# av-savchenko/HSE_FaceRec_tf

Hardware: AMD Instinct MI355X
Metric: faces/sec embedding-extract (MobileNet-192, bs=256) (higher is better)
Workload: dtype f32

## Files before the change

hse_facerec_tf_amd/csrc/dwpw_f16s.hip:

```cpp
#include <type_traits>

#include "common.h"

namespace hsefr {

namespace {

typedef float f32x4 __attribute__((ext_vector_type(4)));
typedef float f32x16 __attribute__((ext_vector_type(16)));
typedef _Float16 f16x4 __attribute__((ext_vector_type(4)));
typedef _Float16 f16x8 __attribute__((ext_vector_type(8)));

struct DwPwSParams {
    const float4* x;
    const float4* wd;
    const float4* dscale;
    const float4* dshift;
    const float* wsplit;
    const float* descale;
    const float* pshift;
    float* y;
    int H, W, C4, KT, OH, OW, Cout, pad_t, pad_l, tiles_w, tiles_h, tiles_n;
    unsigned total;
    float a_scale;
    int reverse;
    int nimg;
    unsigned m_n, m_w, m_h;
    int rows, seam;
    unsigned m_seam;
    unsigned long long* stamps;
};

constexpr int ROWB = 128;
__device__ __forceinline__ int swzb(int row, int chunk) { return row * ROWB + 16 * (chunk ^ ((row >> 1) & 7) ^ ((row & 1) << 2)); }
__device__ __forceinline__ float4 fma4(float4 a, float4 b, float4 c) {
    return make_float4(fmaf(a.x, b.x, c.x), fmaf(a.y, b.y, c.y), fmaf(a.z, b.z, c.z), fmaf(a.w, b.w, c.w));
}
__device__ __forceinline__ float relu6(float v) { return fminf(fmaxf(v, 0.f), 6.f); }
__device__ __forceinline__ unsigned fastdiv(unsigned x, unsigned m) { return m ? __umulhi(x, m) : x; }

template <int STRIDE, int TW, int BN, int OCC, int ACT>
__global__ __launch_bounds__(256, OCC) void dwpw_f16s_kernel(DwPwSParams p) {
    constexpr int TH = 128 / TW;
    constexpr int U = TW * 8;
    constexpr int RG = 256 / U;
    constexpr int RPT = TH / RG;
    static_assert(RPT == 4, "patch shapes 8x16 and 16x8");
    constexpr int WN = BN / 2, NI = WN / 32, BP = BN / 32;
    __shared__ __attribute__((aligned(16))) unsigned char As[128 * ROWB];
    __shared__ __attribute__((aligned(16))) unsigned char Bs[BN * ROWB];

    const int tid = threadIdx.x;
    const int lane = tid & 63, wave = tid >> 6;
    const int wm = wave >> 1, wn = wave & 1;
    const int li = lane & 31, lh = lane >> 5;
    const int srow = tid >> 3, skq = tid & 7;
    const int u = tid % U, tw = u >> 3, c4l = u & 7;
    const int row0 = (tid / U) * RPT;
    const int arow = wm * 64 + li, brow = wn * WN + li;

    for (unsigned t = blockIdx.x; t < p.total; t += gridDim.x) {
        const unsigned lt = xcd_remap_dir(t, p.total, p.reverse);
        const int n0 = (lt % p.tiles_n) * BN;
        const unsigned pt = lt / p.tiles_n;
        const int ow0 = (pt % p.tiles_w) * TW;
        const int oh0 = ((pt / p.tiles_w) % p.tiles_h) * TH;
        const int n = pt / (p.tiles_w * p.tiles_h);

        const int ow = min(ow0 + tw, p.OW - 1);
        const int iw0 = ow * STRIDE - p.pad_l;
        const float ml = iw0 >= 0 ? 1.f : 0.f, mm = (iw0 + 1 >= 0 && iw0 + 1 < p.W) ? 1.f : 0.f, mr = iw0 + 2 < p.W ? 1.f : 0.f;
        const int cl = max(iw0, 0) * p.C4, cm = min(max(iw0 + 1, 0), p.W - 1) * p.C4, cr = min(iw0 + 2, p.W - 1) * p.C4;
        const float4* ximg = p.x + (size_t)n * p.H * p.W * p.C4;
        const int ih0 = (oh0 + row0) * STRIDE - p.pad_t;
        const float* bsrc = p.wsplit + (size_t)(n0 + srow) * p.KT * 32 + 4 * skq;

        f32x16 acc[2][NI];
#pragma unroll
        for (int mi = 0; mi < 2; ++mi)
#pragma unroll
            for (int ni = 0; ni < NI; ++ni)
#pragma unroll
                for (int r = 0; r < 16; ++r) acc[mi][ni][r] = 0.f;

        for (int kc = 0; kc < p.KT; ++kc) {
            f32x4 rb[BP];
#pragma unroll
            for (int q = 0; q < BP; ++q) rb[q] = *(const f32x4*)(bsrc + (size_t)32 * q * p.KT * 32 + kc * 32);
            const int c4 = kc * 8 + c4l;
            const float4* xin = ximg + c4;
            float4 wk[9];
#pragma unroll
            for (int i = 0; i < 9; ++i) {
                const float m = (i % 3 == 0) ? ml : (i % 3 == 1 ? mm : mr);
                const float4 wr = p.wd[i * p.C4 + c4];
                wk[i] = make_float4(wr.x * m, wr.y * m, wr.z * m, wr.w * m);
            }
            const float4 dsc = p.dscale[c4], dsh = p.dshift[c4];
            struct Row { float4 l, m, r; float k; };
            auto load_row = [&](int ih) {
                Row q;
                const int ihc = min(max(ih, 0), p.H - 1);
                const float4* row = xin + (size_t)ihc * p.W * p.C4;
                q.l = row[cl]; q.m = row[cm]; q.r = row[cr];
                q.k = (ih >= 0 && ih < p.H) ? 1.f : 0.f;
                return q;
            };
            auto row_sum = [&](const Row& q, int b) {
                float4 a = make_float4(q.l.x * wk[b].x, q.l.y * wk[b].y, q.l.z * wk[b].z, q.l.w * wk[b].w);
                a = fma4(q.m, wk[b + 1], a);
                return fma4(q.r, wk[b + 2], a);
            };
            f16x4 ohi[RPT], olo[RPT];
            auto emit = [&](int j, const Row& a, const Row& b, const Row& c) {
                const float4 sa = row_sum(a, 0), sb = row_sum(b, 3), sc = row_sum(c, 6);
                float4 s = make_float4(sa.x * a.k, sa.y * a.k, sa.z * a.k, sa.w * a.k);
                s = make_float4(fmaf(sb.x, b.k, s.x), fmaf(sb.y, b.k, s.y), fmaf(sb.z, b.k, s.z), fmaf(sb.w, b.k, s.w));
                s = make_float4(fmaf(sc.x, c.k, s.x), fmaf(sc.y, c.k, s.y), fmaf(sc.z, c.k, s.z), fmaf(sc.w, c.k, s.w));
                const float4 o = fma4(s, dsc, dsh);
                f32x4 v;
                v[0] = relu6(o.x); v[1] = relu6(o.y); v[2] = relu6(o.z); v[3] = relu6(o.w);
                v = v * p.a_scale;
                ohi[j] = __builtin_convertvector(v, f16x4);
                olo[j] = __builtin_convertvector(v - __builtin_convertvector(ohi[j], f32x4), f16x4);
            };
            if (STRIDE == 1) {
                Row r0 = load_row(ih0), r1 = load_row(ih0 + 1), r2 = load_row(ih0 + 2), r3 = load_row(ih0 + 3);
#pragma unroll
                for (int j = 0; j < RPT; ++j) {
                    const Row r4 = load_row(ih0 + j + 4);
                    emit(j, r0, r1, r2);
                    r0 = r1; r1 = r2; r2 = r3; r3 = r4;
                }
            } else {
                Row r0 = load_row(ih0), r1 = load_row(ih0 + 1), r2 = load_row(ih0 + 2);
#pragma unroll
                for (int j = 0; j < RPT; ++j) {
                    const Row n1 = load_row(ih0 + 2 * j + 3), n2 = load_row(ih0 + 2 * j + 4);
                    emit(j, r0, r1, r2);
                    r0 = r2; r1 = n1; r2 = n2;
                }
            }
            __syncthreads();
#pragma unroll
            for (int j = 0; j < RPT; ++j) {
                const int R = (row0 + j) * TW + tw;
                *(f16x4*)(&As[swzb(R, c4l >> 1) + 8 * (c4l & 1)]) = ohi[j];
                *(f16x4*)(&As[swzb(R, 4 + (c4l >> 1)) + 8 * (c4l & 1)]) = olo[j];
            }
#pragma unroll
            for (int q = 0; q < BP; ++q) *(f32x4*)(&Bs[swzb(srow + 32 * q, skq)]) = rb[q];
            __syncthreads();
#pragma unroll
            for (int s = 0; s < 2; ++s) {
                f16x8 ah[2], al[2], bh[NI], bl[NI];
#pragma unroll
                for (int mi = 0; mi < 2; ++mi) {
                    ah[mi] = *(const f16x8*)(&As[swzb(arow + mi * 32, 2 * s + lh)]);
                    al[mi] = *(const f16x8*)(&As[swzb(arow + mi * 32, 4 + 2 * s + lh)]);
                }
#pragma unroll
                for (int ni = 0; ni < NI; ++ni) {
                    bh[ni] = *(const f16x8*)(&Bs[swzb(brow + ni * 32, 2 * s + lh)]);
                    bl[ni] = *(const f16x8*)(&Bs[swzb(brow + ni * 32, 4 + 2 * s + lh)]);
                }
#pragma unroll
                for (int mi = 0; mi < 2; ++mi)
#pragma unroll
                    for (int ni = 0; ni < NI; ++ni) {
                        acc[mi][ni] = __builtin_amdgcn_mfma_f32_32x32x16_f16(al[mi], bh[ni], acc[mi][ni], 0, 0, 0);
                        acc[mi][ni] = __builtin_amdgcn_mfma_f32_32x32x16_f16(ah[mi], bl[ni], acc[mi][ni], 0, 0, 0);
                        acc[mi][ni] = __builtin_amdgcn_mfma_f32_32x32x16_f16(ah[mi], bh[ni], acc[mi][ni], 0, 0, 0);
                    }
            }
        }
        const bool full = oh0 + TH <= p.OH && ow0 + TW <= p.OW;
        float* ybase = p.y + ((size_t)n * p.OH * p.OW) * p.Cout;
#pragma unroll
        for (int ni = 0; ni < NI; ++ni) {
            const int col = n0 + wn * WN + ni * 32 + li;
            const float ds = p.descale[col], sh = p.pshift[col];
#pragma unroll
            for (int mi = 0; mi < 2; ++mi) {
                const int Rb = wm * 64 + mi * 32 + 4 * lh;
                if (full) {
#pragma unroll
                    for (int r = 0; r < 16; ++r) {
                        const int R = Rb + (r & 3) + 8 * (r >> 2);
                        ybase[((size_t)(oh0 + R / TW) * p.OW + ow0 + (R % TW)) * p.Cout + col] = apply_act<ACT>(fmaf(acc[mi][ni][r], ds, sh));
                    }
                } else {
#pragma unroll
                    for (int r = 0; r < 16; ++r) {
                        const int R = Rb + (r & 3) + 8 * (r >> 2);
                        const int oh = oh0 + R / TW, owc = ow0 + (R % TW);
                        if (oh < p.OH && owc < p.OW)
                            ybase[((size_t)oh * p.OW + owc) * p.Cout + col] = apply_act<ACT>(fmaf(acc[mi][ni][r], ds, sh));
                    }
                }
            }
        }
    }
}

constexpr int HALO_B = 192 * 128;
constexpr int CMAX2 = 512;

template <int TW, int BN, int HS, int ACT>
__global__ __launch_bounds__(256 + 64 * (BN == 256 ? 8 : 4), BN == 256 ? 1 : 2) void dwpw3_f16s_kernel(DwPwSParams p) {
    constexpr int NCW = BN == 256 ? 8 : 4;
    constexpr int CWN = NCW / 2;
    constexpr int NTHR = 256 + 64 * NCW;
    constexpr int TH = 128 / TW, HC = TW + 2;
    constexpr int WCAP = 256;
    constexpr int B_ST = BN * ROWB;
    constexpr int B_OFF = HS * HALO_B, A_OFF = B_OFF + 2 * B_ST, W_OFF = A_OFF + 2 * 128 * ROWB, E_OFF = W_OFF + 11 * WCAP * 4;
    constexpr int WN = BN / CWN, NI = WN / 32;
    constexpr int BPW = BN / 8 / NCW;
    static_assert(BPW == 4 && NI == 2, "a consumer's slice of the weight stage is its 4 KB epilogue scratch");
    constexpr bool HALO_BY_CONSUMER = false;
    constexpr int HPW = 24 / (HALO_BY_CONSUMER ? NCW : 4);
    static_assert(E_OFF + 2 * CMAX2 * 4 <= 160 * 1024, "LDS budget");
    __shared__ __attribute__((aligned(1024))) unsigned char smem[E_OFF + 2 * CMAX2 * 4];

    const int tid = threadIdx.x;
    const int lane = tid & 63;
    const int wave = __builtin_amdgcn_readfirstlane(tid >> 6);
    const int C = p.C4 * 4, KT = p.KT;
    {
        float4* wl = (float4*)(smem + W_OFF);
        for (int i = tid; i < 9 * p.C4; i += NTHR) wl[i] = p.wd[i];
        for (int i = tid; i < p.C4; i += NTHR) { wl[9 * p.C4 + i] = p.dscale[i]; wl[10 * p.C4 + i] = p.dshift[i]; }
        float* el = (float*)(smem + E_OFF);
        for (int i = tid; i < p.Cout; i += NTHR) { el[i] = p.descale[i]; el[CMAX2 + i] = p.pshift[i]; }
    }
    const __amdgpu_buffer_rsrc_t rx = make_rsrc(p.x, (long long)p.nimg * p.H * p.W * C * 4);
    const __amdgpu_buffer_rsrc_t rw = make_rsrc(p.wsplit, (long long)p.Cout * C * 4);
    const __amdgpu_buffer_rsrc_t ry = make_rsrc(p.y, (long long)p.nimg * p.OH * p.OW * p.Cout * 4);
    const unsigned OOB = 0xFFFFFFF0u;
    const unsigned nitem = (p.total - blockIdx.x + gridDim.x - 1) / gridDim.x;
    const int nsteps = (int)(nitem * KT);
    struct Item { int n, oh0, ow0, n0; };
    auto decode = [&](unsigned i) {
        const unsigned lt = xcd_remap_dir(blockIdx.x + (i < nitem ? i : nitem - 1) * gridDim.x, p.total, p.reverse);
        Item it;
        const unsigned pt = fastdiv(lt, p.m_n);
        it.n0 = (lt - pt * p.tiles_n) * BN;
        const unsigned pr = fastdiv(pt, p.m_w);
        it.ow0 = (pt - pr * p.tiles_w) * TW;
        it.n = fastdiv(pr, p.m_h);
        it.oh0 = (pr - it.n * p.tiles_h) * TH;
        return it;
    };
    const unsigned lds0 = (unsigned)(unsigned long long)(__attribute__((address_space(3))) unsigned char*)smem;
    auto piece = [&](const __amdgpu_buffer_rsrc_t& r, unsigned lds_addr, unsigned voff, unsigned soff) {
        asm volatile("s_mov_b32 m0, %0\n\ts_nop 0\n\tbuffer_load_dwordx4 %1, %2, %3 offen lds" ::"s"(__builtin_amdgcn_readfirstlane(lds_addr)), "v"(voff),
                     "s"(r), "s"(__builtin_amdgcn_readfirstlane(soff))
                     : "memory", "m0");
    };
    const int hw = HALO_BY_CONSUMER ? wave - 4 : wave & 3;
    unsigned hv[HPW];
    unsigned pf_i = 0;
    int pf_kc = 0, pf_step = 0;
    auto seam_row = [&](const Item& it) {
        return ((int)fastdiv(it.oh0, p.m_seam) + 1) * p.seam - it.oh0;
    };
    auto setup_halo = [&](unsigned i) {
        const Item it = decode(i);
        int zr = 99, lo = 0, hi = p.H;
        if (TW == 8 && p.seam) {
            zr = seam_row(it) + 1;
            lo = it.oh0 + zr - 1 - p.seam;
            hi = p.rows;
        }
        const int nq = (TH + 2 + (zr <= TH ? 1 : 0)) * HC;
#pragma unroll
        for (int j = 0; j < HPW; ++j) {
            const int q = (hw * HPW + j) * 8 + (lane >> 3);
            const int hr = q / HC, hc = q - hr * HC;
            const int ih = it.oh0 - p.pad_t + hr - (hr > zr ? 1 : 0), iw = it.ow0 - p.pad_l + hc;
            const bool ok = q < nq && hr != zr && ih >= lo && ih < hi && iw >= 0 && iw < p.W;
            hv[j] = ok ? ((unsigned)((it.n * p.H + ih) * p.W + iw) * (unsigned)C + 4u * (lane & 7)) * 4u : OOB;
        }
    };
    auto halo_dma = [&]() {
        const unsigned base = lds0 + (pf_step % HS) * HALO_B;
        const unsigned so = (unsigned)pf_kc * 128u;
#pragma unroll
        for (int j = 0; j < HPW; ++j) piece(rx, base + (hw * HPW + j) * 1024, hv[j], so);
        ++pf_step;
        if (++pf_kc == KT) {
            pf_kc = 0;
            setup_halo(++pf_i);
        }
    };
    STEM_STAMP_DECL;

    if (wave < 4) {
        const int quad = tid & 7, col = (tid >> 3) % TW, r0 = 4 * (tid / (8 * TW));
        const unsigned char* hsrc0 = smem + ((r0 * HC + col) * 128 + quad * 16);
        if (!HALO_BY_CONSUMER) {
            setup_halo(0);
#pragma unroll
            for (int i = 0; i < HS - 1; ++i)
                if (i < nsteps) halo_dma();
        }
        asm volatile("s_waitcnt vmcnt(0)" ::: "memory");
        __syncthreads();
        int dkc = 0;
        unsigned di = 0;
        auto seam_shift = [&](unsigned i) { return TW == 8 && p.seam && r0 >= seam_row(decode(i)) ? HC * 128 : 0; };
        int hx = seam_shift(0);
        for (int g = -1; g < nsteps; ++g) {
            const bool issued = !HALO_BY_CONSUMER && pf_step < nsteps;
            if (issued) halo_dma();
            STEM_STAMP(1);
            if (g + 1 < nsteps) {
                const f32x4* wl = (const f32x4*)(smem + W_OFF) + dkc * 8 + quad;
                f32x4 wk[9];
#pragma unroll
                for (int i = 0; i < 9; ++i) wk[i] = wl[i * p.C4];
                const f32x4 dsc = wl[9 * p.C4], dsh = wl[10 * p.C4];
                const unsigned char* hs = hsrc0 + ((g + 1) % HS) * HALO_B + hx;
                unsigned char* At = smem + A_OFF + ((g + 1) & 1) * (128 * ROWB);
                f32x4 h[6][3];
#pragma unroll
                for (int a = 0; a < 6; ++a)
#pragma unroll
                    for (int b = 0; b < 3; ++b) h[a][b] = *(const f32x4*)(hs + (a * HC + b) * 128);
                auto row_sum = [&](int a, int b) {
                    f32x4 t = h[a][0] * wk[b];
                    t = __builtin_elementwise_fma(h[a][1], wk[b + 1], t);
                    return __builtin_elementwise_fma(h[a][2], wk[b + 2], t);
                };
#pragma unroll
                for (int j = 0; j < 4; ++j) {
                    const f32x4 sa = row_sum(j, 0), sb = row_sum(j + 1, 3), sc = row_sum(j + 2, 6);
                    const f32x4 sacc = (sa + sb) + sc;
                    const f32x4 o = __builtin_elementwise_fma(sacc, dsc, dsh);
                    f32x4 v;
#pragma unroll
                    for (int e = 0; e < 4; ++e) v[e] = relu6(o[e]);
                    v = v * p.a_scale;
                    const f16x4 hi = __builtin_convertvector(v, f16x4);
                    const f16x4 lo = __builtin_convertvector(v - __builtin_convertvector(hi, f32x4), f16x4);
                    const int R = (r0 + j) * TW + col;
                    *(f16x4*)(At + swzb(R, quad >> 1) + 8 * (quad & 1)) = hi;
                    *(f16x4*)(At + swzb(R, 4 + (quad >> 1)) + 8 * (quad & 1)) = lo;
                }
                if (++dkc == KT) { dkc = 0; hx = seam_shift(++di); STEM_STAMP_COUNT; }
// ... 272 lines not shown
                const float fb = rk[2 * j + 1], fc = rk[2 * j + 2];
                f32x4 sum = sa * rk[2 * j];
                sum = __builtin_elementwise_fma(sb, f32x4{fb, fb, fb, fb}, sum);
                sum = __builtin_elementwise_fma(sc, f32x4{fc, fc, fc, fc}, sum);
                const f32x4 o = __builtin_elementwise_fma(sum, dsc, dsh);
                f32x4 v;
#pragma unroll
                for (int e = 0; e < 4; ++e) v[e] = relu6(o[e]);
                v = v * p.a_scale;
                const f16x4 hi = __builtin_convertvector(v, f16x4);
                const f16x4 lo = __builtin_convertvector(v - __builtin_convertvector(hi, f32x4), f16x4);
                const int R = (row0 + j) * S2_T + col;
                *(f16x4*)(At + swzb(R, quad >> 1) + 8 * (quad & 1)) = hi;
                *(f16x4*)(At + swzb(R, 4 + (quad >> 1)) + 8 * (quad & 1)) = lo;
            }
            if (++ckc == S2_KT) {
                ckc = 0;
                setup_factors(++ci);
            }
        };
        setup_loads(0);
        setup_factors(0);
        gload(S0());
        for (int t = 0; t < nsteps; t += 2) {
            gload(S1());
            produce(S0(), smem + S2_A_OFF);
            __syncthreads();
            gload(S0());
            produce(S1(), smem + S2_A_OFF + S2_A_ST);
            __syncthreads();
        }
    } else {
        const int cw = wave - 4;
        const int li = lane & 31, lh = lane >> 5;
        const int brow = cw * 64 + li;
        const int erow = lane >> 3, ech = lane & 7;
        f32x16 acc[2][2];
        auto zero_acc = [&]() {
#pragma unroll
            for (int mi = 0; mi < 2; ++mi)
#pragma unroll
                for (int ni = 0; ni < 2; ++ni)
#pragma unroll
                    for (int r = 0; r < 16; ++r) acc[mi][ni][r] = 0.f;
        };
        auto epilogue = [&](const Item& cur) {
            unsigned char* scr = smem + S2_S_OFF + cw * S2_SCR;
            const float* el = (const float*)(smem + S2_E_OFF);
            unsigned sv[2][2][2];
#pragma unroll
            for (int mi = 0; mi < 2; ++mi)
#pragma unroll
                for (int hb = 0; hb < 2; ++hb)
#pragma unroll
                    for (int i = 0; i < 2; ++i) {
                        const int R = mi * 32 + hb * 16 + erow + 8 * i;
                        const int oh = cur.oh0 + R / S2_T, ow = cur.ow0 + R % S2_T;
                        sv[mi][hb][i] = (oh < p.OH && ow < p.OW)
                                            ? ((unsigned)((cur.n * p.OH + oh) * p.OW + ow) * (unsigned)S2_COUT + (unsigned)(cw * 64 + 4 * ech)) * 4u
                                            : OOB;
                    }
#pragma unroll
            for (int ni = 0; ni < 2; ++ni) {
                const int nl = cw * 64 + ni * 32 + 4 * ech;
                const f32x4 ds = *(const f32x4*)(el + nl), sh = *(const f32x4*)(el + S2_COUT + nl);
#pragma unroll
                for (int mi = 0; mi < 2; ++mi)
#pragma unroll
                    for (int hb = 0; hb < 2; ++hb) {
                        if ((li >> 4) == hb) {
#pragma unroll
                            for (int j = 0; j < 4; ++j) {
                                f32x4 v;
#pragma unroll
                                for (int e = 0; e < 4; ++e) v[e] = acc[mi][ni][4 * j + e];
                                *(f32x4*)(scr + (li & 15) * 128 + 16 * ((2 * j + lh) ^ (li & 7))) = v;
                            }
                        }
                        f32x4 rv[2];
#pragma unroll
                        for (int i = 0; i < 2; ++i) {
                            const int r = erow + 8 * i;
                            rv[i] = *(const f32x4*)(scr + r * 128 + 16 * (ech ^ (r & 7)));
                        }
#pragma unroll
                        for (int i = 0; i < 2; ++i) {
                            const f32x4 z = __builtin_elementwise_fma(rv[i], ds, sh);
                            f32x4 o;
#pragma unroll
                            for (int e = 0; e < 4; ++e) o[e] = apply_act<ACT>(z[e]);
                            bstore16_welded(o, ry, sv[mi][hb][i], __builtin_amdgcn_readfirstlane((unsigned)(ni * 32) * 4u));
                        }
                    }
            }
        };
        zero_acc();
        Item cur = decode(0);
        unsigned ci = 0;
        int ckc = 0;
        bool pending = false;
        for (int g = 0; g < nsteps; ++g) {
            if (pending) {
                epilogue(cur);
                zero_acc();
                cur = decode(++ci);
                pending = false;
            }
            __syncthreads();
            const unsigned char* As = smem + S2_A_OFF + (g & 1) * S2_A_ST;
            const unsigned char* Bs = smem + ckc * S2_B_ST;
#pragma unroll
            for (int s = 0; s < 2; ++s) {
                f16x8 ah[2], al[2], bh[2], bl[2];
#pragma unroll
                for (int mi = 0; mi < 2; ++mi) {
                    ah[mi] = *(const f16x8*)(As + swzb(li + mi * 32, 2 * s + lh));
                    al[mi] = *(const f16x8*)(As + swzb(li + mi * 32, 4 + 2 * s + lh));
                }
#pragma unroll
                for (int ni = 0; ni < 2; ++ni) {
                    bh[ni] = *(const f16x8*)(Bs + swzb(brow + ni * 32, 2 * s + lh));
                    bl[ni] = *(const f16x8*)(Bs + swzb(brow + ni * 32, 4 + 2 * s + lh));
                }
#pragma unroll
                for (int mi = 0; mi < 2; ++mi)
#pragma unroll
                    for (int ni = 0; ni < 2; ++ni) {
                        acc[mi][ni] = __builtin_amdgcn_mfma_f32_32x32x16_f16(bh[ni], al[mi], acc[mi][ni], 0, 0, 0);
                        acc[mi][ni] = __builtin_amdgcn_mfma_f32_32x32x16_f16(bl[ni], ah[mi], acc[mi][ni], 0, 0, 0);
                        acc[mi][ni] = __builtin_amdgcn_mfma_f32_32x32x16_f16(bh[ni], ah[mi], acc[mi][ni], 0, 0, 0);
                    }
            }
            if (++ckc == S2_KT) { ckc = 0; pending = true; }
        }
        epilogue(cur);
    }
}

HSEFR_KNOB(g_s2_off, "dwpw_s2_off", 0);
HSEFR_KNOB(g_tw, "dwpws_tw", 0);
HSEFR_KNOB(g_bn, "dwpws_bn", 0);

template <int STRIDE, int TW, int BN, int OCC>
int launch_t(DwPwSParams& p, int n, int act, hipStream_t s) {
    constexpr int TH = 128 / TW;
    p.tiles_w = (p.OW + TW - 1) / TW;
    p.tiles_h = (p.OH + TH - 1) / TH;
    p.tiles_n = p.Cout / BN;
    const long long total = (long long)n * p.tiles_w * p.tiles_h * p.tiles_n;
    HSEFR_REQUIRE(total < (1ll << 31), HSEFR_ERR_UNSUPPORTED, "dwpw_f16split: grid too large");
    p.total = (unsigned)total;
    const unsigned cap = 256u * OCC;
    const unsigned g = p.total < cap ? p.total : cap;
#define HSEFR_DWPWS(A) HSEFR_LAUNCH((dwpw_f16s_kernel<STRIDE, TW, BN, OCC, A>), dim3(g), dim3(256), 0, s, p)
    if (act == HSEFR_ACT_RELU6) HSEFR_DWPWS(HSEFR_ACT_RELU6);
    else if (act == HSEFR_ACT_RELU) HSEFR_DWPWS(HSEFR_ACT_RELU);
    else if (act == HSEFR_ACT_NONE) HSEFR_DWPWS(HSEFR_ACT_NONE);
    else { set_error("dwpw_f16split: act %d", act); return HSEFR_ERR_UNSUPPORTED; }
#undef HSEFR_DWPWS
    return launch_status("dwpw_f16split");
}

template <int STRIDE, int TW>
int launch_bn(DwPwSParams& p, int n, int bn, int act, hipStream_t s) {
    if (bn == 64) return launch_t<STRIDE, TW, 64, 2>(p, n, act, s);
#ifdef HSEFR_DEV
    if (bn == 256) return launch_t<STRIDE, TW, 256, 2>(p, n, act, s);
#endif
    return launch_t<STRIDE, TW, 128, 2>(p, n, act, s);
}

template <int TW, int BN, int HS>
int launch_v3(DwPwSParams& p, int n, int act, bool strip, hipStream_t s) {
    constexpr int TH = 128 / TW;
    auto magic = [](unsigned d) { return d == 1 ? 0u : (unsigned)((0x100000000ull + d - 1) / d); };
    if (strip) {
        HSEFR_REQUIRE(TW == 8 && (long long)n * p.OH * p.OH < (1ll << 32), HSEFR_ERR_UNSUPPORTED, "dwpw_f16split: strip tiling");
        p.rows = n * p.OH; p.seam = p.OH; p.m_seam = magic(p.OH);
        n = 1;
    }
    p.tiles_w = (p.OW + TW - 1) / TW;
    p.tiles_h = (p.rows + TH - 1) / TH;
    p.tiles_n = p.Cout / BN;
    const long long total = (long long)n * p.tiles_w * p.tiles_h * p.tiles_n;
    HSEFR_REQUIRE(total < (1ll << 31) / 16, HSEFR_ERR_UNSUPPORTED, "dwpw_f16split: grid too large");
    p.total = (unsigned)total;
    p.m_n = magic(p.tiles_n); p.m_w = magic(p.tiles_w); p.m_h = magic(p.tiles_h);
    HSEFR_REQUIRE(total * (long long)(p.tiles_n > p.tiles_w ? (p.tiles_n > p.tiles_h ? p.tiles_n : p.tiles_h) : (p.tiles_w > p.tiles_h ? p.tiles_w : p.tiles_h)) < (1ll << 32),
                  HSEFR_ERR_UNSUPPORTED, "dwpw_f16split: grid too large for the quotient multipliers");
    const unsigned g = p.total < 256u ? p.total : 256u;
#define HSEFR_DWPW3(A) HSEFR_LAUNCH((dwpw3_f16s_kernel<TW, BN, HS, A>), dim3(g), dim3(256 + 64 * (BN == 256 ? 8 : 4)), 0, s, p)
    if (act == HSEFR_ACT_RELU6) HSEFR_DWPW3(HSEFR_ACT_RELU6);
    else if (act == HSEFR_ACT_RELU) HSEFR_DWPW3(HSEFR_ACT_RELU);
    else if (act == HSEFR_ACT_NONE) HSEFR_DWPW3(HSEFR_ACT_NONE);
    else { set_error("dwpw_f16split: act %d", act); return HSEFR_ERR_UNSUPPORTED; }
#undef HSEFR_DWPW3
    return launch_status("dwpw_f16split");
}

int launch_s2(DwPwSParams& p, int n, int act, hipStream_t s) {
    p.tiles_w = (p.OW + S2_T - 1) / S2_T;
    p.tiles_h = (p.OH + S2_T - 1) / S2_T;
    p.tiles_n = 1;
    const long long total = (long long)n * p.tiles_w * p.tiles_h;
    HSEFR_REQUIRE(total < (1ll << 31) / 16, HSEFR_ERR_UNSUPPORTED, "dwpw_f16split: grid too large");
    p.total = (unsigned)total;
    auto magic = [](unsigned d) { return d == 1 ? 0u : (unsigned)((0x100000000ull + d - 1) / d); };
    p.m_n = 0; p.m_w = magic(p.tiles_w); p.m_h = magic(p.tiles_h);
    HSEFR_REQUIRE(total * (long long)(p.tiles_w > p.tiles_h ? p.tiles_w : p.tiles_h) < (1ll << 32), HSEFR_ERR_UNSUPPORTED,
                  "dwpw_f16split: grid too large for the quotient multipliers");
    const unsigned g = p.total < S2_GRID ? p.total : S2_GRID;
#define HSEFR_DWPWS2(A) HSEFR_LAUNCH((dwpws2_f16s_kernel<A>), dim3(g), dim3(512), 0, s, p)
    if (act == HSEFR_ACT_RELU6) HSEFR_DWPWS2(HSEFR_ACT_RELU6);
    else if (act == HSEFR_ACT_RELU) HSEFR_DWPWS2(HSEFR_ACT_RELU);
    else if (act == HSEFR_ACT_NONE) HSEFR_DWPWS2(HSEFR_ACT_NONE);
    else { set_error("dwpw_f16split: act %d", act); return HSEFR_ERR_UNSUPPORTED; }
#undef HSEFR_DWPWS2
    return launch_status("dwpw_f16split");
}

}


bool dwpw_s2_off() { return g_s2_off != 0; }

bool dwpw_s2_covered(int c, int cout, int stride) { return stride == 2 && c == S2_C && cout == S2_COUT; }

bool dwpw_f16s_supported(int c, int cout, int stride) {
    return c > 0 && c % 32 == 0 && cout > 0 && cout % 64 == 0 && (stride == 1 || stride == 2);
}

int launch_dwpw_f16s(const float* x, const float* wd, const float* dscale, const float* dshift, const void* wsplit,
                     const float* descale, const float* pshift, float* y, int n, int h, int w, int c, int stride, int pad_t,
                     int pad_l, int oh, int ow, int cout, int a_log2, int act, hipStream_t s) {
    HSEFR_REQUIRE(dwpw_f16s_supported(c, cout, stride), HSEFR_ERR_UNSUPPORTED,
                  "dwpw_f16split: c=%d cout=%d stride=%d not covered (c %% 32, cout %% 64, stride 1|2)", c, cout, stride);
    HSEFR_REQUIRE(n >= 0 && h > 0 && w > 0 && oh > 0 && ow > 0, HSEFR_ERR_INVALID, "dwpw_f16split: bad shape");
    HSEFR_REQUIRE(a_log2 > 0 && a_log2 <= 12, HSEFR_ERR_INVALID, "dwpw_f16split: a_log2=%d (the depthwise result is in [0,6]: 1..12)", a_log2);
    if (n == 0) return HSEFR_OK;
    DwPwSParams p;
    p.x = (const float4*)x; p.wd = (const float4*)wd; p.dscale = (const float4*)dscale; p.dshift = (const float4*)dshift;
    p.wsplit = (const float*)wsplit; p.descale = descale; p.pshift = pshift; p.y = y;
    p.H = h; p.W = w; p.C4 = c / 4; p.KT = c / 32; p.OH = oh; p.OW = ow; p.Cout = cout; p.pad_t = pad_t; p.pad_l = pad_l;
    p.a_scale = ldexpf(1.f, a_log2);
    p.reverse = sweep_reverse();
    p.nimg = n;
    p.rows = oh; p.seam = 0; p.m_seam = 0;
    p.stamps = nullptr;
#ifdef HSEFR_STEM_STAMPS
    p.stamps = stamp_buffer(s);
#endif
    const long long in_bytes = (long long)n * h * w * c * 4, out_bytes = (long long)n * oh * ow * cout * 4;
    if (stride == 1 && c <= 256 && cout <= CMAX2 && cout % 128 == 0 && in_bytes < (1ll << 32) - 16 && out_bytes < (1ll << 32) - 16) {
        auto padded = [&](int tw) { const int th = 128 / tw; return (long long)((ow + tw - 1) / tw * tw) * ((oh + th - 1) / th * th); };
        int tw = padded(16) <= padded(8) ? 16 : 8;
        if (g_tw == 8 || g_tw == 16) tw = g_tw;
        const bool strip = g_tw != 16 && oh % 4 == 0 && oh >= 16 && h == oh && pad_t == 1 && (long long)n * oh * oh < (1ll << 32) &&
                           (long long)((ow + 7) / 8 * 8) * (((long long)n * oh + 15) / 16 * 16) < n * padded(tw);
        if (strip) tw = 8;
        int bn = cout % 256 == 0 ? 256 : 128;
        if ((g_bn == 128 || g_bn == 256) && cout % g_bn == 0) bn = g_bn;
        if (bn == 256) return tw == 16 ? launch_v3<16, 256, 2>(p, n, act, false, s) : launch_v3<8, 256, 2>(p, n, act, strip, s);
        return tw == 16 ? launch_v3<16, 128, 3>(p, n, act, false, s) : launch_v3<8, 128, 3>(p, n, act, strip, s);
    }
    if (dwpw_s2_covered(c, cout, stride) && !g_s2_off && in_bytes < (1ll << 32) - 16 && out_bytes < (1ll << 32) - 16)
        return launch_s2(p, n, act, s);
    int bn = cout % 128 == 0 ? 128 : 64;
    if (g_bn && cout % g_bn == 0) bn = g_bn;
    int tw = (ow % 16 == 0 || ow % 8 != 0) ? 16 : 8;
    if (ow <= 8) tw = 8;
    if (g_tw == 8 || g_tw == 16) tw = g_tw;
    if (stride == 1) return tw == 16 ? launch_bn<1, 16>(p, n, bn, act, s) : launch_bn<1, 8>(p, n, bn, act, s);
    return tw == 16 ? launch_bn<2, 16>(p, n, bn, act, s) : launch_bn<2, 8>(p, n, bn, act, s);
}

}
```

hse_facerec_tf_amd/csrc/pwblk_stream.hip:

```cpp
#include "common.h"

#ifndef PB_ABLATE
#define PB_ABLATE 0
#endif
namespace hsefr {

namespace {

typedef float f32x4 __attribute__((ext_vector_type(4)));
typedef float f32x16 __attribute__((ext_vector_type(16)));
typedef _Float16 f16x4 __attribute__((ext_vector_type(4)));
typedef _Float16 f16x8 __attribute__((ext_vector_type(8)));

constexpr int PB_CIN = 64, PB_C = 128, PB_COUT = 128;
constexpr int PB_WMAX = 48;
constexpr unsigned PB_GRID = 256;
constexpr int PB_ROWB = 128;
constexpr int PB_CELLB = PB_C * 4;
constexpr int PB_RING = (PB_WMAX + 2) * PB_CELLB;
constexpr int PB_KT = PB_WMAX * PB_ROWB;
constexpr int PB_A2 = (PB_CIN / 32) * PB_KT, PB_A3 = (PB_C / 32) * PB_KT;
constexpr int PB_A2_OFF = 2 * PB_RING, PB_A3_OFF = PB_A2_OFF + 2 * PB_A2, PB_S_OFF = PB_A3_OFF + 2 * PB_A3;
constexpr int PB_ITEMS = 64;
constexpr int PB_E_OFF = PB_S_OFF + 4 * 8192, PB_T_OFF = PB_E_OFF + 2 * PB_C * 4, PB_LDS = PB_T_OFF + PB_ITEMS * 16;
static_assert(PB_LDS <= 160 * 1024, "LDS budget");

struct PwBlkParams {
    const float* x;
    const float* w2;
    const float* ds2;
    const float* sh2;
    const f32x4* wd;
    const f32x4* dscale;
    const f32x4* dshift;
    const float* w3;
    const float* ds3;
    const float* sh3;
    float* y;
    int nimg, H, W, S;
    unsigned total;
    float a_scale2, a_scale3;
    int reverse;
    int act;
    hsefr_udiv kS;
};

__device__ __forceinline__ int swzb(int row, int chunk) { return row * PB_ROWB + 16 * (chunk ^ ((row >> 1) & 7) ^ ((row & 1) << 2)); }
__device__ __forceinline__ float relu6(float v) { return fminf(fmaxf(v, 0.f), 6.f); }
__device__ __forceinline__ int ringb(int cell, int chunk) { return cell * PB_CELLB + 16 * (chunk ^ (cell & 7)); }

constexpr int NB = 2;

__global__ __launch_bounds__(512, 1) void pwblk_stream_f16s_kernel(PwBlkParams p) {
    __shared__ __attribute__((aligned(1024))) unsigned char smem[PB_LDS];
    const int tid = threadIdx.x;
    const int lane = tid & 63;
    const int wave = __builtin_amdgcn_readfirstlane(tid >> 6);
    const int H = p.H, W = p.W;
    const unsigned OOB = 0xFFFFFFF0u;
    for (int i = tid; i < 2 * PB_RING / 16; i += 512) ((f32x4*)smem)[i] = f32x4{0.f, 0.f, 0.f, 0.f};
    {
        float* el = (float*)(smem + PB_E_OFF);
        if (tid < PB_C) { el[tid] = p.ds2[tid]; el[PB_C + tid] = p.sh2[tid]; }
    }
    const unsigned nitem = (p.total - blockIdx.x + gridDim.x - 1) / gridDim.x;
    int* itab = (int*)(smem + PB_T_OFF);
    if (tid < (int)nitem) {
        const unsigned lt = xcd_remap_dir(blockIdx.x + (unsigned)tid * gridDim.x, p.total, p.reverse);
        const bool one = p.S == 1;
        const unsigned n = one ? lt : hsefr_udiv_do(lt, p.kS), seg = lt - n * (unsigned)p.S;
        const int r0 = one ? 0 : (int)hsefr_udiv_do(seg * (unsigned)H, p.kS);
        itab[4 * tid] = (int)n;
        itab[4 * tid + 1] = r0;
        itab[4 * tid + 2] = (one ? H : (int)hsefr_udiv_do((seg + 1u) * (unsigned)H, p.kS)) - r0 + 2;
    }
    __syncthreads();
    struct Cur { unsigned i; int s, R, n, r0; };
    auto open = [&](Cur& c) {
        const int* e = itab + 4 * (c.i < nitem ? c.i : nitem - 1);
        c.n = __builtin_amdgcn_readfirstlane(e[0]);
        c.r0 = __builtin_amdgcn_readfirstlane(e[1]);
        c.R = __builtin_amdgcn_readfirstlane(e[2]);
        c.s = 0;
    };
    auto next = [&](Cur& c) {
        if (++c.s == c.R) { ++c.i; open(c); }
    };
    int nflat = 0;
    for (unsigned i = 0; i < nitem; ++i) nflat += __builtin_amdgcn_readfirstlane(itab[4 * i + 2]);
    const int nsteps = nflat + 3;
    __syncthreads();

    if (wave < 4) {
        const __amdgpu_buffer_rsrc_t rx = make_rsrc(p.x, (long long)p.nimg * H * W * PB_CIN * 4);
        unsigned xv[3];
        int a2o[3];
#pragma unroll
        for (int j = 0; j < 3; ++j) {
            const int i = tid + 256 * j;
            xv[j] = i < W * 16 ? (unsigned)i * 16u : OOB;
            const int cq = i & 15, skq = cq & 7;
            a2o[j] = (cq >> 3) * PB_KT + swzb(i >> 4, skq >> 1) + 8 * (skq & 1);
        }
        f32x4 xr[3];
        Cur cl;
        cl.i = 0;
        open(cl);
        auto gload = [&]() {
            const int q = cl.r0 - 1 + cl.s;
            const bool ok = q >= 0 && q < H;
            const unsigned so = __builtin_amdgcn_readfirstlane(ok ? (unsigned)((cl.n * H + q) * W) * (unsigned)(PB_CIN * 4) : 0u);
#pragma unroll
            for (int j = 0; j < 3; ++j) xr[j] = bload16(rx, ok ? xv[j] : OOB, so);
            next(cl);
        };
        auto split = [&](unsigned char* At) {
#pragma unroll
            for (int j = 0; j < 3; ++j) {
                const f32x4 v = xr[j] * p.a_scale2;
                const f16x4 hi = __builtin_convertvector(v, f16x4);
                const f16x4 lo = __builtin_convertvector(v - __builtin_convertvector(hi, f32x4), f16x4);
                *(f16x4*)(At + a2o[j]) = hi;
                *(f16x4*)(At + (a2o[j] ^ 64)) = lo;
            }
        };
        const int quad = tid & 31, pg = tid >> 5;
        f32x4 wk[9];
#pragma unroll
        for (int i = 0; i < 9; ++i) wk[i] = p.wd[i * (PB_C / 4) + quad];
        const f32x4 dsc = p.dscale[quad], dsh = p.dshift[quad];
        int ro[3];
#pragma unroll
        for (int t = 0; t < 3; ++t) ro[t] = ringb(pg + t, quad);
        const int a3e = (quad >> 3) * PB_KT + swzb(pg, (quad & 7) >> 1) + 8 * (quad & 1);
        f32x4 top[6], mid[6];
#pragma unroll
        for (int j = 0; j < 6; ++j) top[j] = mid[j] = f32x4{0.f, 0.f, 0.f, 0.f};
        auto depthwise = [&](const unsigned char* rs, unsigned char* At) {
#pragma unroll
            for (int j = 0; j < 6; ++j) {
                const f32x4 h0 = *(const f32x4*)(rs + ro[0] + j * 8 * PB_CELLB), h1 = *(const f32x4*)(rs + ro[1] + j * 8 * PB_CELLB),
                            h2 = *(const f32x4*)(rs + ro[2] + j * 8 * PB_CELLB);
                auto row_sum = [&](int b) {
                    f32x4 t = h0 * wk[b];
                    t = __builtin_elementwise_fma(h1, wk[b + 1], t);
                    return __builtin_elementwise_fma(h2, wk[b + 2], t);
                };
                const f32x4 sa = row_sum(0), sb = row_sum(3), sc = row_sum(6);
                const f32x4 sacc = mid[j] + sc;
                mid[j] = top[j] + sb;
                top[j] = sa;
                const f32x4 o = __builtin_elementwise_fma(sacc, dsc, dsh);
                f32x4 v;
#pragma unroll
                for (int e = 0; e < 4; ++e) v[e] = relu6(o[e]);
                v = v * p.a_scale3;
                const f16x4 hi = __builtin_convertvector(v, f16x4);
                const f16x4 lo = __builtin_convertvector(v - __builtin_convertvector(hi, f32x4), f16x4);
                const int ao = (a3e ^ (64 * (j & 1))) + j * 8 * PB_ROWB;
                *(f16x4*)(At + ao) = hi;
                *(f16x4*)(At + (ao ^ 64)) = lo;
            }
        };
        gload();
#pragma nounroll
        for (int g = 0; g < nsteps; ++g) {
            if (!(PB_ABLATE & 4)) {
                if (g < nflat) split(smem + PB_A2_OFF + (g & 1) * PB_A2);
                gload();
            }
            if (!(PB_ABLATE & 2) && g >= 2 && g < nflat + 2) depthwise(smem + (g & 1) * PB_RING, smem + PB_A3_OFF + (g & 1) * PB_A3);
            __syncthreads();
        }
    } else {
        const int cw = wave - 4;
        const int li = lane & 31, lh = lane >> 5;
        const int erow = lane >> 3, ech = lane & 7;
        const __amdgpu_buffer_rsrc_t ry = make_rsrc(p.y, (long long)p.nimg * H * W * PB_COUT * 4);
        f16x8 w2h[4], w2l[4], w3h[8], w3l[8];
        {
            const unsigned char* r2 = (const unsigned char*)p.w2 + (size_t)(32 * cw + li) * (PB_CIN * 4);
            const unsigned char* r3 = (const unsigned char*)p.w3 + (size_t)(32 * cw + li) * (PB_C * 4);
#pragma unroll
            for (int s = 0; s < 4; ++s) {
                w2h[s] = *(const f16x8*)(r2 + (s >> 1) * 128 + (2 * (s & 1) + lh) * 16);
                w2l[s] = *(const f16x8*)(r2 + (s >> 1) * 128 + 64 + (2 * (s & 1) + lh) * 16);
            }
#pragma unroll
            for (int s = 0; s < 8; ++s) {
                w3h[s] = *(const f16x8*)(r3 + (s >> 1) * 128 + (2 * (s & 1) + lh) * 16);
                w3l[s] = *(const f16x8*)(r3 + (s >> 1) * 128 + 64 + (2 * (s & 1) + lh) * 16);
            }
        }
        f32x4 ds3 = *(const f32x4*)(p.ds3 + 32 * cw + 4 * ech), sh3 = *(const f32x4*)(p.sh3 + 32 * cw + 4 * ech);
#pragma unroll
        for (int s = 0; s < 4; ++s) asm volatile("" : "+v"(w2h[s]), "+v"(w2l[s]));
#pragma unroll
        for (int s = 0; s < 8; ++s) asm volatile("" : "+v"(w3h[s]), "+v"(w3l[s]));
        asm volatile("" : "+v"(ds3), "+v"(sh3));
        const float* el = (const float*)(smem + PB_E_OFF);
        unsigned char* scr = smem + PB_S_OFF + cw * 8192;
        Cur c1, c3;
        c1.i = 0;
        open(c1);
        c3 = c1;
        f32x16 acc2[NB], acc3[NB];
        f16x8 fh[2][NB], fl[2][NB];
        auto zero = [&](f32x16* acc) {
#pragma unroll
            for (int b = 0; b < NB; ++b)
#pragma unroll
                for (int r = 0; r < 16; ++r) acc[b][r] = 0.f;
        };
        auto fragments = [&](const unsigned char* St, int s, int buf) {
            const unsigned char* row = St + (s >> 1) * PB_KT;
#pragma unroll
            for (int b = 0; b < NB; ++b) {
                fh[buf][b] = *(const f16x8*)(row + swzb(b * 32 + li, 2 * (s & 1) + lh));
                fl[buf][b] = *(const f16x8*)(row + swzb(b * 32 + li, 4 + 2 * (s & 1) + lh));
            }
        };
        auto mfmas = [&](f32x16* acc, const f16x8& wh, const f16x8& wl, int buf) {
#pragma unroll
            for (int b = 0; b < NB; ++b) {
                acc[b] = __builtin_amdgcn_mfma_f32_32x32x16_f16(wh, fl[buf][b], acc[b], 0, 0, 0);
                acc[b] = __builtin_amdgcn_mfma_f32_32x32x16_f16(wl, fh[buf][b], acc[b], 0, 0, 0);
                acc[b] = __builtin_amdgcn_mfma_f32_32x32x16_f16(wh, fh[buf][b], acc[b], 0, 0, 0);
            }
        };
        auto product3 = [&](const unsigned char* St) {
            zero(acc3);
            fragments(St, 0, 0);
#pragma unroll
            for (int s = 0; s < 8; ++s) {
                if (s + 1 < 8) fragments(St, s + 1, (s + 1) & 1);
                mfmas(acc3, w3h[s], w3l[s], s & 1);
            }
        };
        unsigned sv[NB][4];
        f32x4 rv[4];
        auto out_park = [&](int b) {
#pragma unroll
            for (int j = 0; j < 4; ++j) {
                f32x4 v;
#pragma unroll
                for (int e = 0; e < 4; ++e) v[e] = acc3[b][4 * j + e];
                *(f32x4*)(scr + b * 4096 + li * 128 + 16 * ((2 * j + lh) ^ (li & 7))) = v;
            }
        };
        auto out_fetch = [&](int b) {
#pragma unroll
            for (int i = 0; i < 4; ++i) {
                const int rr = erow + 8 * i;
                rv[i] = *(const f32x4*)(scr + b * 4096 + rr * 128 + 16 * (ech ^ (rr & 7)));
            }
        };
        auto out_store = [&](int b) {
            f32x4 o[4];
#pragma unroll
            for (int i = 0; i < 4; ++i) o[i] = __builtin_elementwise_fma(rv[i], ds3, sh3);
            if (p.act == HSEFR_ACT_RELU6) {
#pragma unroll
                for (int i = 0; i < 4; ++i)
#pragma unroll
                    for (int e = 0; e < 4; ++e) o[i][e] = apply_act<HSEFR_ACT_RELU6>(o[i][e]);
            } else if (p.act == HSEFR_ACT_RELU) {
#pragma unroll
                for (int i = 0; i < 4; ++i)
#pragma unroll
                    for (int e = 0; e < 4; ++e) o[i][e] = apply_act<HSEFR_ACT_RELU>(o[i][e]);
            }
#pragma unroll
            for (int i = 0; i < 4; ++i)
                if (!(PB_ABLATE & 8)) bstore16_welded(o[i], ry, sv[b][i], 0u);
        };
#pragma nounroll
        for (int g = 0; g < nsteps; ++g) {
            const int par = (g + 1) & 1;
            const bool emit = !(PB_ABLATE & 1) && g >= 3 && g < nflat + 3 && c3.s >= 2;
            const bool feed = !(PB_ABLATE & 1) && g >= 1 && g < nflat + 1;
            const int q = c1.r0 - 1 + c1.s;
            const bool inside = feed && q >= 0 && q < H;
            unsigned char* slot = smem + par * PB_RING;
            const unsigned char* A2s = smem + PB_A2_OFF + par * PB_A2;
            if (emit) {
                const int r = c3.r0 + c3.s - 2;
#pragma unroll
                for (int b = 0; b < NB; ++b)
#pragma unroll
                    for (int i = 0; i < 4; ++i) {
                        const int px = b * 32 + erow + 8 * i;
                        sv[b][i] = px < W ? ((unsigned)((c3.n * H + r) * W + px) * (unsigned)PB_COUT + (unsigned)(32 * cw + 4 * ech)) * 4u : OOB;
                    }
                product3(smem + PB_A3_OFF + par * PB_A3);
                out_park(0);
                out_park(1);
            }
            if (inside) {
                zero(acc2);
                fragments(A2s, 0, 0);
                fragments(A2s, 1, 1);
                mfmas(acc2, w2h[0], w2l[0], 0);
            }
            if (emit) out_fetch(0);
            if (inside) {
                fragments(A2s, 2, 0);
                mfmas(acc2, w2h[1], w2l[1], 1);
            }
            if (emit) { out_store(0); out_fetch(1); }
            if (inside) {
                fragments(A2s, 3, 1);
                mfmas(acc2, w2h[2], w2l[2], 0);
            }
            if (emit) out_store(1);
            if (inside) mfmas(acc2, w2h[3], w2l[3], 1);
            if (inside) {
                f32x4 ds[4], sh[4];
#pragma unroll
                for (int j = 0; j < 4; ++j) {
                    ds[j] = *(const f32x4*)(el + 32 * cw + 8 * j + 4 * lh);
                    sh[j] = *(const f32x4*)(el + PB_C + 32 * cw + 8 * j + 4 * lh);
                }
#pragma unroll
                for (int b = 0; b < NB; ++b)
#pragma unroll
                    for (int j = 0; j < 4; ++j) {
                        f32x4 v;
#pragma unroll
                        for (int e = 0; e < 4; ++e) v[e] = relu6(fmaf(acc2[b][4 * j + e], ds[j][e], sh[j][e]));
                        if (b * 32 + li < W) *(f32x4*)(slot + ringb(b * 32 + li + 1, 8 * cw + 2 * j + lh)) = v;
                    }
            } else if (feed) {
#pragma unroll
                for (int b = 0; b < NB; ++b)
#pragma unroll
                    for (int j = 0; j < 4; ++j)
                        if (b * 32 + li < W) *(f32x4*)(slot + ringb(b * 32 + li + 1, 8 * cw + 2 * j + lh)) = f32x4{0.f, 0.f, 0.f, 0.f};
            }
            if (!(PB_ABLATE & 1) && g >= 3 && g < nflat + 3) next(c3);
            if (feed) next(c1);
            __syncthreads();
        }
    }
}

}

bool pwblk_covered(int cin, int cmid, int cout, int w) { return cin == PB_CIN && cmid == PB_C && cout == PB_COUT && w >= 1 && w <= PB_WMAX; }

int launch_pwblk_f16s(const float* x, const void* w2split, const float* descale2, const float* shift2, const float* wd, const float* dscale,
                      const float* dshift, const void* w3split, const float* descale3, const float* shift3, float* y, int n, int h, int w,
                      int a_log2, int a_log2_blk, int act, int segs, hipStream_t s) {
    HSEFR_REQUIRE(n >= 0 && h > 0 && w > 0 && w <= PB_WMAX, HSEFR_ERR_UNSUPPORTED, "pwblk_f16split: map %d x %d not covered (rows of at most %d pixels)",
                  h, w, PB_WMAX);
    HSEFR_REQUIRE(a_log2 > 0 && a_log2 <= 12 && a_log2_blk > 0 && a_log2_blk <= 12, HSEFR_ERR_INVALID, "pwblk_f16split: a_log2=%d / %d (1..12)", a_log2,
                  a_log2_blk);
    HSEFR_REQUIRE(segs >= 0, HSEFR_ERR_INVALID, "pwblk_f16split: segs=%d", segs);
    if (n == 0) return HSEFR_OK;
    HSEFR_REQUIRE((long long)n * h * w * PB_COUT * 4 < (1ll << 32) - 16, HSEFR_ERR_UNSUPPORTED, "pwblk_f16split: tensors beyond 4 GB");
    PwBlkParams p;
    p.x = x; p.w2 = (const float*)w2split; p.ds2 = descale2; p.sh2 = shift2;
    p.wd = (const f32x4*)wd; p.dscale = (const f32x4*)dscale; p.dshift = (const f32x4*)dshift;
    p.w3 = (const float*)w3split; p.ds3 = descale3; p.sh3 = shift3; p.y = y;
    p.nimg = n; p.H = h; p.W = w;
    int S = segs;
    if (S == 0) {
        const int fill = (int)((PB_GRID + (unsigned)n - 1) / (unsigned)n), most = h / 4 > 1 ? h / 4 : 1;
        S = fill < most ? fill : most;
    }
    p.S = S < h ? S : h;
    if (p.S > PB_ITEMS) p.S = PB_ITEMS;
    p.kS = hsefr_udiv_make(p.S >= 2 ? (unsigned)p.S : 2u);
    p.a_scale2 = ldexpf(1.f, a_log2);
    p.a_scale3 = ldexpf(1.f, a_log2_blk);
    p.reverse = sweep_reverse();
    HSEFR_REQUIRE(act == HSEFR_ACT_RELU6 || act == HSEFR_ACT_RELU || act == HSEFR_ACT_NONE, HSEFR_ERR_UNSUPPORTED, "pwblk_f16split: act %d", act);
    p.act = act;
    const int per = (int)(PB_GRID * PB_ITEMS) / p.S;
    for (int n0 = 0; n0 < n; n0 += per) {
        p.nimg = n - n0 < per ? n - n0 : per;
        p.x = x + (size_t)n0 * h * w * PB_CIN;
        p.y = y + (size_t)n0 * h * w * PB_COUT;
        p.total = (unsigned)p.nimg * (unsigned)p.S;
        const unsigned g = p.total < PB_GRID ? p.total : PB_GRID;
        HSEFR_LAUNCH(pwblk_stream_f16s_kernel, dim3(g), dim3(512), 0, s, p);
    }
    return launch_status("pwblk_f16split");
}

}
```

Measured before the change: 262,100.

## Deepen pwblk global-load pipeline, template on width-bucket and activation

Measured after the change: 264,300 (median of 6 runs). Within noise of the previous version (+0.8%).

```diff
diff --git a/hse_facerec_tf_amd/csrc/dwpw_f16s.hip b/hse_facerec_tf_amd/csrc/dwpw_f16s.hip
--- a/hse_facerec_tf_amd/csrc/dwpw_f16s.hip
+++ b/hse_facerec_tf_amd/csrc/dwpw_f16s.hip
@@ -27,7 +27,10 @@
     int nimg;
     unsigned m_n, m_w, m_h;
     int rows, seam;
-    unsigned m_seam;
+    union {
+        unsigned m_seam;
+        int act;
+    };
     unsigned long long* stamps;
 };
 
@@ -39,7 +42,7 @@
 __device__ __forceinline__ float relu6(float v) { return fminf(fmaxf(v, 0.f), 6.f); }
 __device__ __forceinline__ unsigned fastdiv(unsigned x, unsigned m) { return m ? __umulhi(x, m) : x; }
 
-template <int STRIDE, int TW, int BN, int OCC, int ACT>
+template <int STRIDE, int TW, int BN, int OCC>
 __global__ __launch_bounds__(256, OCC) void dwpw_f16s_kernel(DwPwSParams p) {
     constexpr int TH = 128 / TW;
     constexpr int U = TW * 8;
@@ -183,19 +186,28 @@
 #pragma unroll
             for (int mi = 0; mi < 2; ++mi) {
                 const int Rb = wm * 64 + mi * 32 + 4 * lh;
+                float o[16];
+#pragma unroll
+                for (int r = 0; r < 16; ++r) o[r] = fmaf(acc[mi][ni][r], ds, sh);
+                if (p.act == HSEFR_ACT_RELU6) {
+#pragma unroll
+                    for (int r = 0; r < 16; ++r) o[r] = apply_act<HSEFR_ACT_RELU6>(o[r]);
+                } else if (p.act == HSEFR_ACT_RELU) {
+#pragma unroll
+                    for (int r = 0; r < 16; ++r) o[r] = apply_act<HSEFR_ACT_RELU>(o[r]);
+                }
                 if (full) {
 #pragma unroll
                     for (int r = 0; r < 16; ++r) {
                         const int R = Rb + (r & 3) + 8 * (r >> 2);
-                        ybase[((size_t)(oh0 + R / TW) * p.OW + ow0 + (R % TW)) * p.Cout + col] = apply_act<ACT>(fmaf(acc[mi][ni][r], ds, sh));
+                        ybase[((size_t)(oh0 + R / TW) * p.OW + ow0 + (R % TW)) * p.Cout + col] = o[r];
                     }
                 } else {
 #pragma unroll
                     for (int r = 0; r < 16; ++r) {
                         const int R = Rb + (r & 3) + 8 * (r >> 2);
                         const int oh = oh0 + R / TW, owc = ow0 + (R % TW);
-                        if (oh < p.OH && owc < p.OW)
-                            ybase[((size_t)oh * p.OW + owc) * p.Cout + col] = apply_act<ACT>(fmaf(acc[mi][ni][r], ds, sh));
+                        if (oh < p.OH && owc < p.OW) ybase[((size_t)oh * p.OW + owc) * p.Cout + col] = o[r];
                     }
                 }
             }
@@ -774,12 +786,9 @@
     p.total = (unsigned)total;
     const unsigned cap = 256u * OCC;
     const unsigned g = p.total < cap ? p.total : cap;
-#define HSEFR_DWPWS(A) HSEFR_LAUNCH((dwpw_f16s_kernel<STRIDE, TW, BN, OCC, A>), dim3(g), dim3(256), 0, s, p)
-    if (act == HSEFR_ACT_RELU6) HSEFR_DWPWS(HSEFR_ACT_RELU6);
-    else if (act == HSEFR_ACT_RELU) HSEFR_DWPWS(HSEFR_ACT_RELU);
-    else if (act == HSEFR_ACT_NONE) HSEFR_DWPWS(HSEFR_ACT_NONE);
-    else { set_error("dwpw_f16split: act %d", act); return HSEFR_ERR_UNSUPPORTED; }
-#undef HSEFR_DWPWS
+    HSEFR_REQUIRE(act == HSEFR_ACT_RELU6 || act == HSEFR_ACT_RELU || act == HSEFR_ACT_NONE, HSEFR_ERR_UNSUPPORTED, "dwpw_f16split: act %d", act);
+    p.act = act;
+    HSEFR_LAUNCH((dwpw_f16s_kernel<STRIDE, TW, BN, OCC>), dim3(g), dim3(256), 0, s, p);
     return launch_status("dwpw_f16split");
 }
 
diff --git a/hse_facerec_tf_amd/csrc/pwblk_stream.hip b/hse_facerec_tf_amd/csrc/pwblk_stream.hip
--- a/hse_facerec_tf_amd/csrc/pwblk_stream.hip
+++ b/hse_facerec_tf_amd/csrc/pwblk_stream.hip
@@ -1,3 +1,5 @@
+#include <type_traits>
+
 #include "common.h"
 
 #ifndef PB_ABLATE
@@ -41,7 +43,6 @@
     unsigned total;
     float a_scale2, a_scale3;
     int reverse;
-    int act;
     hsefr_udiv kS;
 };
 
@@ -49,8 +50,7 @@
 __device__ __forceinline__ float relu6(float v) { return fminf(fmaxf(v, 0.f), 6.f); }
 __device__ __forceinline__ int ringb(int cell, int chunk) { return cell * PB_CELLB + 16 * (chunk ^ (cell & 7)); }
 
-constexpr int NB = 2;
-
+template <int NB, int ACT>
 __global__ __launch_bounds__(512, 1) void pwblk_stream_f16s_kernel(PwBlkParams p) {
     __shared__ __attribute__((aligned(1024))) unsigned char smem[PB_LDS];
     const int tid = threadIdx.x;
@@ -88,36 +88,40 @@
     };
     int nflat = 0;
     for (unsigned i = 0; i < nitem; ++i) nflat += __builtin_amdgcn_readfirstlane(itab[4 * i + 2]);
-    const int nsteps = nflat + 3;
+    const int nsteps = (nflat + 3 + 3) & ~3;
     __syncthreads();
 
     if (wave < 4) {
-        const __amdgpu_buffer_rsrc_t rx = make_rsrc(p.x, (long long)p.nimg * H * W * PB_CIN * 4);
-        unsigned xv[3];
-        int a2o[3];
-#pragma unroll
-        for (int j = 0; j < 3; ++j) {
+        const long long xbytes = (long long)p.nimg * H * W * PB_CIN * 4;
+        constexpr int NL = NB == 1 ? 2 : 3, NJ = NB == 1 ? 4 : 6;
+        unsigned xv[NL];
+        int a2o[NL];
+#pragma unroll
+        for (int j = 0; j < NL; ++j) {
             const int i = tid + 256 * j;
             xv[j] = i < W * 16 ? (unsigned)i * 16u : OOB;
             const int cq = i & 15, skq = cq & 7;
             a2o[j] = (cq >> 3) * PB_KT + swzb(i >> 4, skq >> 1) + 8 * (skq & 1);
         }
-        f32x4 xr[3];
+        f32x4 xr[4][NL];
         Cur cl;
         cl.i = 0;
         open(cl);
-        auto gload = [&]() {
+        auto gload = [&](auto SET) {
+            constexpr int S = decltype(SET)::value;
             const int q = cl.r0 - 1 + cl.s;
-            const bool ok = q >= 0 && q < H;
+            const bool ok = cl.i < nitem && q >= 0 && q < H;
             const unsigned so = __builtin_amdgcn_readfirstlane(ok ? (unsigned)((cl.n * H + q) * W) * (unsigned)(PB_CIN * 4) : 0u);
-#pragma unroll
-            for (int j = 0; j < 3; ++j) xr[j] = bload16(rx, ok ? xv[j] : OOB, so);
+            const __amdgpu_buffer_rsrc_t r = make_rsrc(p.x, ok ? xbytes : 0);
+#pragma unroll
+            for (int j = 0; j < NL; ++j) xr[S][j] = bload16(r, xv[j], so);
             next(cl);
         };
-        auto split = [&](unsigned char* At) {
-#pragma unroll
-            for (int j = 0; j < 3; ++j) {
-                const f32x4 v = xr[j] * p.a_scale2;
+        auto split = [&](auto SET, unsigned char* At) {
+            constexpr int S = decltype(SET)::value;
+#pragma unroll
+            for (int j = 0; j < NL; ++j) {
+                const f32x4 v = xr[S][j] * p.a_scale2;
                 const f16x4 hi = __builtin_convertvector(v, f16x4);
                 const f16x4 lo = __builtin_convertvector(v - __builtin_convertvector(hi, f32x4), f16x4);
                 *(f16x4*)(At + a2o[j]) = hi;
@@ -133,12 +137,12 @@
 #pragma unroll
         for (int t = 0; t < 3; ++t) ro[t] = ringb(pg + t, quad);
         const int a3e = (quad >> 3) * PB_KT + swzb(pg, (quad & 7) >> 1) + 8 * (quad & 1);
-        f32x4 top[6], mid[6];
-#pragma unroll
-        for (int j = 0; j < 6; ++j) top[j] = mid[j] = f32x4{0.f, 0.f, 0.f, 0.f};
+        f32x4 top[NJ], mid[NJ];
+#pragma unroll
+        for (int j = 0; j < NJ; ++j) top[j] = mid[j] = f32x4{0.f, 0.f, 0.f, 0.f};
         auto depthwise = [&](const unsigned char* rs, unsigned char* At) {
 #pragma unroll
-            for (int j = 0; j < 6; ++j) {
+            for (int j = 0; j < NJ; ++j) {
                 const f32x4 h0 = *(const f32x4*)(rs + ro[0] + j * 8 * PB_CELLB), h1 = *(const f32x4*)(rs + ro[1] + j * 8 * PB_CELLB),
                             h2 = *(const f32x4*)(rs + ro[2] + j * 8 * PB_CELLB);
                 auto row_sum = [&](int b) {
@@ -162,15 +166,28 @@
                 *(f16x4*)(At + (ao ^ 64)) = lo;
             }
         };
-        gload();
+#pragma unroll
+        for (int i = 0; i < 9; ++i) asm volatile("" : "+v"(wk[i]));
+        typedef std::integral_constant<int, 0> S0;
+        typedef std::integral_constant<int, 1> S1;
+        typedef std::integral_constant<int, 2> S2;
+        typedef std::integral_constant<int, 3> S3;
+        auto step = [&](int g, auto SET) {
+            constexpr int S = decltype(SET)::value;
+            if (!(PB_ABLATE & 4)) {
+                gload(std::integral_constant<int, (S + 3) & 3>{});
+                split(SET, smem + PB_A2_OFF + (S & 1) * PB_A2);
+            }
+            if (!(PB_ABLATE & 2) && g >= 2 && g < nflat + 2) depthwise(smem + (S & 1) * PB_RING, smem + PB_A3_OFF + (S & 1) * PB_A3);
+            __syncthreads();
+        };
+        if (!(PB_ABLATE & 4)) { gload(S0{}); gload(S1{}); gload(S2{}); }
 #pragma nounroll
-        for (int g = 0; g < nsteps; ++g) {
-            if (!(PB_ABLATE & 4)) {
-                if (g < nflat) split(smem + PB_A2_OFF + (g & 1) * PB_A2);
-                gload();
-            }
-            if (!(PB_ABLATE & 2) && g >= 2 && g < nflat + 2) depthwise(smem + (g & 1) * PB_RING, smem + PB_A3_OFF + (g & 1) * PB_A3);
-            __syncthreads();
+        for (int g = 0; g < nsteps; g += 4) {
+            step(g, S0{});
+            step(g + 1, S1{});
+            step(g + 2, S2{});
+            step(g + 3, S3{});
         }
     } else {
         const int cw = wave - 4;
@@ -259,17 +276,10 @@
             f32x4 o[4];
 #pragma unroll
             for (int i = 0; i < 4; ++i) o[i] = __builtin_elementwise_fma(rv[i], ds3, sh3);
-            if (p.act == HSEFR_ACT_RELU6) {
-#pragma unroll
-                for (int i = 0; i < 4; ++i)
-#pragma unroll
-                    for (int e = 0; e < 4; ++e) o[i][e] = apply_act<HSEFR_ACT_RELU6>(o[i][e]);
-            } else if (p.act == HSEFR_ACT_RELU) {
-#pragma unroll
-                for (int i = 0; i < 4; ++i)
-#pragma unroll
-                    for (int e = 0; e < 4; ++e) o[i][e] = apply_act<HSEFR_ACT_RELU>(o[i][e]);
-            }
+#pragma unroll
+            for (int i = 0; i < 4; ++i)
+#pragma unroll
+                for (int e = 0; e < 4; ++e) o[i][e] = apply_act<ACT>(o[i][e]);
 #pragma unroll
             for (int i = 0; i < 4; ++i)
                 if (!(PB_ABLATE & 8)) bstore16_welded(o[i], ry, sv[b][i], 0u);
@@ -293,8 +303,8 @@
                         sv[b][i] = px < W ? ((unsigned)((c3.n * H + r) * W + px) * (unsigned)PB_COUT + (unsigned)(32 * cw + 4 * ech)) * 4u : OOB;
                     }
                 product3(smem + PB_A3_OFF + par * PB_A3);
-                out_park(0);
-                out_park(1);
+#pragma unroll
+                for (int b = 0; b < NB; ++b) out_park(b);
             }
             if (inside) {
                 zero(acc2);
@@ -307,12 +317,12 @@
                 fragments(A2s, 2, 0);
                 mfmas(acc2, w2h[1], w2l[1], 1);
             }
-            if (emit) { out_store(0); out_fetch(1); }
+            if (emit) { out_store(0); if (NB > 1) out_fetch(1); }
             if (inside) {
                 fragments(A2s, 3, 1);
                 mfmas(acc2, w2h[2], w2l[2], 0);
             }
-            if (emit) out_store(1);
+            if (NB > 1 && emit) out_store(1);
             if (inside) mfmas(acc2, w2h[3], w2l[3], 1);
             if (inside) {
                 f32x4 ds[4], sh[4];
@@ -375,7 +385,6 @@
     p.a_scale3 = ldexpf(1.f, a_log2_blk);
     p.reverse = sweep_reverse();
     HSEFR_REQUIRE(act == HSEFR_ACT_RELU6 || act == HSEFR_ACT_RELU || act == HSEFR_ACT_NONE, HSEFR_ERR_UNSUPPORTED, "pwblk_f16split: act %d", act);
-    p.act = act;
     const int per = (int)(PB_GRID * PB_ITEMS) / p.S;
     for (int n0 = 0; n0 < n; n0 += per) {
         p.nimg = n - n0 < per ? n - n0 : per;
@@ -383,7 +392,13 @@
         p.y = y + (size_t)n0 * h * w * PB_COUT;
         p.total = (unsigned)p.nimg * (unsigned)p.S;
         const unsigned g = p.total < PB_GRID ? p.total : PB_GRID;
-        HSEFR_LAUNCH(pwblk_stream_f16s_kernel, dim3(g), dim3(512), 0, s, p);
+#define HSEFR_PWBLK(B, A) HSEFR_LAUNCH((pwblk_stream_f16s_kernel<B, A>), dim3(g), dim3(512), 0, s, p)
+#define HSEFR_PWBLK_B(A) do { if (w <= 32) HSEFR_PWBLK(1, A); else HSEFR_PWBLK(2, A); } while (0)
+        if (act == HSEFR_ACT_RELU6) HSEFR_PWBLK_B(HSEFR_ACT_RELU6);
+        else if (act == HSEFR_ACT_RELU) HSEFR_PWBLK_B(HSEFR_ACT_RELU);
+        else HSEFR_PWBLK_B(HSEFR_ACT_NONE);
+#undef HSEFR_PWBLK_B
+#undef HSEFR_PWBLK
     }
     return launch_status("pwblk_f16split");
 }
```
